# optuna/optuna

Hardware: NVIDIA H100
Metric: TPE suggestions/sec at 100k-trial history, 32 params (higher is better)
Workload: dtype f64

## Files before the change

### optuna_b200/csrc/tpe_kernels.cuh

```cuda
#pragma once
#include <cooperative_groups.h>

#include <type_traits>

#include "tpe_common.cuh"
#include "tpe_math.cuh"
#include "mt_jump_table.inc"

namespace tpe {

__global__ void k_rowok(const double* __restrict__ X, int64_t n, int32_t pall, const ColMeta* __restrict__ cols,
                        int32_t pc, uint8_t* __restrict__ ok) {
  for (int64_t i = blockIdx.x * (int64_t)blockDim.x + threadIdx.x; i < n; i += (int64_t)gridDim.x * blockDim.x) {
    bool good = true;
    for (int j = 0; j < pc; ++j) {
      const double v = X[i * pall + cols[j].src];
      good = good && (v == v);
    }
    ok[i] = good ? 1 : 0;
  }
}

struct SplitWork {
  int cat_count[4];
// ... 1102 lines not shown
  __device__ __forceinline__ void push_sync(double L) {
    const bool hit = L > thr;
    b3 = hit ? b2 : b3;
    b2 = hit ? b1 : b2;
    b1 = hit ? b0 : b1;
    b0 = hit ? L : b0;
    cnt += hit ? 1 : 0;
    if (__any_sync(0xffffffffu, cnt == 4)) flush();
  }
};

template <int PB, int PS, int RC, int NT, int TK, int ST, bool PAIR, int MINB>
__global__ void __launch_bounds__(NT, MINB)
k_logpdf_fast(const void* __restrict__ tab_v, const double* __restrict__ cst, int64_t Kf,
              const double2* __restrict__ colprm, const double* __restrict__ xT, int64_t ct_stride, int64_t kps,
              double lse_skip, double2* __restrict__ part) {
  static_assert(PB % PS == 0 && RC % PS == 0, "bad tiling");
  static_assert(!PAIR || PS == 1, "PAIR tables are not split over lanes");
  constexpr int PL = PB / PS;
  constexpr int RL = RC / PS;
  constexpr int GW = 32 / PS;
  constexpr int CW = GW * RC;
  using Elem = typename std::conditional<PAIR, double2, double>::type;
  constexpr int ES = PAIR ? 16 : 8;
  extern __shared__ __align__(128) unsigned char smem_raw[];
  Elem* tiles = reinterpret_cast<Elem*>(smem_raw);
  double* csts = reinterpret_cast<double*>(smem_raw + (size_t)ST * TK * PB * ES);
  uint64_t* full = reinterpret_cast<uint64_t*>(csts + (size_t)ST * TK);
  const Elem* tab = reinterpret_cast<const Elem*>(tab_v);
  const int tid = threadIdx.x;
  const int lane = tid & 31;
  const int h = lane % PS;
  const int g = lane / PS;
  const int64_t k0 = blockIdx.y * kps;
  const int64_t k1 = (k0 + kps < Kf) ? k0 + kps : Kf;
  const int ntiles = (k1 > k0) ? (int)((k1 - k0 + TK - 1) / TK) : 0;
  const int64_t wbase = (int64_t)blockIdx.x * ((NT / 32) * CW) + (int64_t)(tid >> 5) * CW;

  if (tid == 0) {
    for (int s = 0; s < ST; ++s) mbar_init(&full[s], 1);
    mbar_fence_init();
    LseAcc::skip() = lse_skip;
  }
  __syncthreads();

  auto issue = [&](int t) {
    const int st = t % ST;
    const int64_t ks = k0 + (int64_t)t * TK;
    const int tk = (int)((k1 - ks < TK) ? (k1 - ks) : TK);
    const uint32_t b_tile = (uint32_t)(((size_t)tk * PB * ES + 15) & ~(size_t)15);
    const uint32_t b_cst = (uint32_t)(((tk + 1) & ~1) * 8);
    fence_proxy_async();
    mbar_expect_tx(&full[st], b_tile + b_cst);
    bulk_g2s(tiles + (size_t)st * TK * PB, tab + ks * PB, b_tile, &full[st]);
    bulk_g2s(csts + (size_t)st * TK, cst + ks, b_cst, &full[st]);
  };
  if (tid == 0) {
    for (int t = 0; t < ST - 1 && t < ntiles; ++t) issue(t);
  }

  double x[RC][PL];
#pragma unroll
  for (int p = 0; p < PL; ++p) {
    const int slot = (PL == 1) ? h : 2 * ((p >> 1) * PS + h) + (p & 1);
    const double2 cp = colprm[slot];
#pragma unroll
    for (int r = 0; r < RC; ++r) {
      const int64_t ct = wbase + (int64_t)r * GW + g;
      x[r][p] = (xT[(int64_t)slot * ct_stride + ct] - cp.x) * cp.y;
    }
  }
  LseAcc acc[RL];
#pragma unroll
  for (int r = 0; r < RL; ++r) acc[r].init();

  for (int t = 0; t < ntiles; ++t) {
    const int st = t % ST;
    if (tid == 0 && t + ST - 1 < ntiles) issue(t + ST - 1);
    mbar_wait(&full[st], (uint32_t)((t / ST) & 1));
    const int64_t ks = k0 + (int64_t)t * TK;
    const int tk = (int)((k1 - ks < TK) ? (k1 - ks) : TK);
    const Elem* tile = tiles + (size_t)st * TK * PB;
    const double* ctile = csts + (size_t)st * TK;
    for (int kk = 0; kk < tk; ++kk) {
      double a0[RC], a1[RC];
#pragma unroll
      for (int r = 0; r < RC; ++r) {
        a0[r] = 0.0;
        a1[r] = 0.0;
      }
      if constexpr (PAIR) {
        const double2* row = reinterpret_cast<const double2*>(tile) + (size_t)kk * PB;
#pragma unroll
        for (int p = 0; p < PL; ++p) {
          const double2 v = row[p];
#pragma unroll
          for (int r = 0; r < RC; ++r) {
            const double d = fma(x[r][p], v.y, -v.x);
            if (p & 1) a1[r] = fma(d, d, a1[r]);
            else a0[r] = fma(d, d, a0[r]);
          }
        }
      } else if constexpr (PL == 1) {
        const double v = reinterpret_cast<const double*>(tile)[(size_t)kk * PB + h];
#pragma unroll
        for (int r = 0; r < RC; ++r) {
          const double d = x[r][0] - v;
          a0[r] = d * d;
        }
      } else {
        const double2* row =
            reinterpret_cast<const double2*>(reinterpret_cast<const double*>(tile) + (size_t)kk * PB) + h;
#pragma unroll
        for (int q = 0; q < PL / 2; ++q) {
          const double2 v = row[q * PS];
#pragma unroll
          for (int r = 0; r < RC; ++r) {
            const double d0 = x[r][2 * q] - v.x;
            const double d1 = x[r][2 * q + 1] - v.y;
            a0[r] = fma(d0, d0, a0[r]);
            a1[r] = fma(d1, d1, a1[r]);
          }
        }
      }
      double sum[RC];
#pragma unroll
      for (int r = 0; r < RC; ++r) sum[r] = a0[r] + a1[r];
      if constexpr (PS == 2) {
#pragma unroll
        for (int r = 0; r < RL; ++r) {
          const double mine = h ? sum[RL + r] : sum[r];
          const double send = h ? sum[r] : sum[RL + r];
          sum[r] = mine + __shfl_xor_sync(0xffffffffu, send, 1);
        }
      } else if constexpr (PS == 4) {
        double half[RC / 2];
#pragma unroll
        for (int r = 0; r < RC / 2; ++r) {
          const double mine = (h & 2) ? sum[RC / 2 + r] : sum[r];
          const double send = (h & 2) ? sum[r] : sum[RC / 2 + r];
          half[r] = mine + __shfl_xor_sync(0xffffffffu, send, 2);
        }
#pragma unroll
        for (int r = 0; r < RL; ++r) {
          const double mine = (h & 1) ? half[RL + r] : half[r];
          const double send = (h & 1) ? half[r] : half[RL + r];
          sum[r] = mine + __shfl_xor_sync(0xffffffffu, send, 1);
        }
      }
      const double c = ctile[kk];
#pragma unroll
      for (int r = 0; r < RL; ++r) acc[r].push_sync(fma(-0.5, sum[r], c));
    }
    __syncthreads();
  }
#pragma unroll
  for (int r = 0; r < RL; ++r) acc[r].flush();
#pragma unroll
  for (int r = 0; r < RL; ++r) {
    const int64_t ct = wbase + (int64_t)(h * RL + r) * GW + g;
    part[blockIdx.y * ct_stride + ct] = make_double2(acc[r].m, acc[r].s);
  }
}

__device__ __forceinline__ float ex2_approx(float x) {
  float y;
  asm("ex2.approx.ftz.f32 %0, %1;" : "=f"(y) : "f"(x));
  return y;
}
__device__ __forceinline__ double uni_exp(double x, const double* __restrict__ tab64) {
  const double t = fma(x, 92.332482616893656768, 6755399441055744.0);
  const int ni = __double2loint(t);
  const double nf = t - 6755399441055744.0;
  double r = fma(nf, -1.08304246932675596327e-02, x);
  r = fma(nf, -2.98158582698529328128e-12, r);
  double p = 8.33333333333333333333e-03;
  p = fma(p, r, 4.16666666666666666667e-02);
  p = fma(p, r, 1.66666666666666666667e-01);
  p = fma(p, r, 0.5);
  p = fma(p, r, 1.0);
  p = fma(p, r, 1.0);
  const double y = tab64[ni & 63] * p;
  return __hiloint2double(__double2hiint(y) + ((ni >> 6) << 20), __double2loint(y));
}

constexpr double kRefMove = 48.0;
__device__ __forceinline__ unsigned long long ld_relaxed_gpu(const unsigned long long* p) {
  unsigned long long v;
  asm volatile("ld.relaxed.gpu.global.u64 %0, [%1];" : "=l"(v) : "l"(p));
  return v;
}
struct LseRef {
  double R, s, base;
  float ffar;
  float thn;
  unsigned wp;
  __device__ __forceinline__ void init(unsigned slot0) {
    R = -INFINITY; s = 0.0; base = -INFINITY;
    ffar = 0.0f; thn = -INFINITY; wp = slot0;
  }
  __device__ __forceinline__ void rebase(double nb, float tnear, const double* e64) {
    if (__any_sync(0xffffffffu, nb > R + kRefMove)) {
      const bool mv = nb > R + kRefMove;
      const double f = uni_exp(fmax(R - nb, -700.0), e64);
      s = mv ? (s + (double)ffar) * f : s;
      ffar = mv ? 0.0f : ffar;
      R = mv ? nb : R;
    }
    base = nb;
    const float d = __double2float_rn(base - R);
    thn = (R == -INFINITY) ? -INFINITY : d - tnear;
  }
  template <int RS>
  __device__ __forceinline__ void flush(const double* ring, float tnear, const double* e64) {
    const unsigned slot0 = (unsigned)__cvta_generic_to_shared(ring);
    const int cnt = parked<RS>(slot0);
    const int n = __reduce_max_sync(0xffffffffu, cnt);
    double nb = base;
    for (int i = 0; i < n; ++i) {
      const double v = ring[i * RS];
      nb = (i < cnt && v > nb) ? v : nb;
    }
    rebase(nb, tnear, e64);
    double sum = 0.0;
    for (int i = 0; i < n; ++i) {
      const double e = uni_exp(fmax(ring[i * RS] - R, -700.0), e64);
      sum += (i < cnt) ? e : 0.0;
    }
    s += sum;
    wp = slot0;
  }
  template <int RS>
  __device__ __forceinline__ void park(double L, bool near) {
    asm volatile("{\n\t.reg .pred p;\n\tsetp.ne.u32 p, %2, 0;\n\t@p st.shared.f64 [%0], %1;\n\t}"
                 :: "r"(wp), "d"(L), "r"((unsigned)near) : "memory");
    wp += near ? RS * 8 : 0;
  }
  template <int RS>
  __device__ __forceinline__ int parked(unsigned slot0) const { return (int)((wp - slot0) / (RS * 8)); }
  __device__ __forceinline__ void roll() {
    s += (double)ffar;
    ffar = 0.0f;
  }
  __device__ __forceinline__ void sync_global(unsigned long long* slot, unsigned long long& pend, float tnear,
                                              const double* e64) {
    const double seen = from_order_bits(pend);
    pend = ld_relaxed_gpu(slot);
    if (base > seen) atomicMax(slot, static_cast<unsigned long long>(order_bits(base)));
    if (__any_sync(0xffffffffu, seen > base)) rebase(fmax(base, seen), tnear, e64);
  }
  __device__ __forceinline__ bool classify(double L, float gap, float& add, int& nfar) const {
    const float df = __double2float_rn(L - R);
    const bool near = df > thn;
    const bool far = !near && df > thn - gap;
    const float e = ex2_approx(df * 1.44269504f);
    add += far ? e : 0.0f;
    nfar += far ? 1 : 0;
    return near;
  }
  __device__ __forceinline__ double2 result(const double* e64) const {
    return make_double2(base, s * uni_exp(fmax(R - base, -700.0), e64));
  }
};

__device__ __forceinline__ void dmma_8x8x4(double& d0, double& d1, double a, double b) {
  asm volatile("mma.sync.aligned.m8n8k4.row.col.f64.f64.f64.f64 {%0,%1}, {%2}, {%3}, {%0,%1};"
               : "+d"(d0), "+d"(d1)
               : "d"(a), "d"(b));
}
__device__ __forceinline__ void dmma_16x8x8(double& d0, double& d1, double& d2, double& d3, double a0, double a1,
                                            double a2, double a3, double b0, double b1) {
  asm volatile("mma.sync.aligned.m16n8k8.row.col.f64.f64.f64.f64 {%0,%1,%2,%3}, {%4,%5,%6,%7}, {%8,%9}, {%0,%1,%2,%3};"
               : "+d"(d0), "+d"(d1), "+d"(d2), "+d"(d3)
               : "d"(a0), "d"(a1), "d"(a2), "d"(a3), "d"(b0), "d"(b1));
}
template <int PB, int M, int KG, int NT, int TK, int ST, int MINB>
struct MmaSmem {
  static constexpr size_t stages = (size_t)ST * TK * PB * 8 + (size_t)ST * TK * 8 + (size_t)ST * 16;
  static constexpr int NVG = 2 * KG;
  static constexpr int RS = (NT / 32) * M * 32;
  static constexpr size_t kSm = 228 * 1024, kCta = 1024 + 64 * 8;
  static constexpr size_t ctas_ = kSm / (stages + kCta);
  static constexpr size_t ctas = ctas_ < (size_t)MINB ? ctas_ : (size_t)MINB;
  static constexpr size_t fit = (kSm / ctas - kCta - stages) / (RS * 8);
  static constexpr int cap = (2 * NVG > 8) ? 2 * NVG : 8;
  static constexpr int D = (fit < (size_t)cap) ? (int)fit : cap;
  static_assert(D >= NVG, "the near-term ring does not fit beside the TMA stages: fewer stages or a shorter tile");
  static constexpr size_t bytes = stages + (size_t)D * RS * 8;
};

#ifdef TPE_LAB
__device__ unsigned long long g_mma_lab_count[5];
#endif

template <int PB, int M, int KG, int NT, int TK, int ST, int MINB, int DBG = 0>
__global__ void __launch_bounds__(NT, MINB)
k_logpdf_mma(const double* __restrict__ tabm, const double* __restrict__ ckk, int64_t Kfp,
             const double2* __restrict__ colprm, const double* __restrict__ xT, int64_t ct_stride, int64_t kps,
             double lse_skip, double2* __restrict__ part, unsigned long long* __restrict__ gmax,
             double lse_near) {
  static_assert(PB % 8 == 0 && TK % (8 * KG) == 0 && (M == 1 || M % 2 == 0), "bad tiling");
  constexpr int NI = PB / 4;
  constexpr int CW = 8 * M;
  extern __shared__ __align__(128) unsigned char smem_raw[];
  __shared__ double s_e64[64];
  double* tiles = reinterpret_cast<double*>(smem_raw);
  double* csts = tiles + (size_t)ST * TK * PB;
  uint64_t* full = reinterpret_cast<uint64_t*>(csts + (size_t)ST * TK);
  uint64_t* empty = full + ST;
  using SM = MmaSmem<PB, M, KG, NT, TK, ST, MINB>;
  double* ring = reinterpret_cast<double*>(empty + ST) + (threadIdx.x >> 5) * M * 32 + (threadIdx.x & 31);
  const int tid = threadIdx.x;
  const int lane = tid & 31;
  const int g = lane >> 2, q = lane & 3;
  const int64_t k0 = blockIdx.y * kps;
  const int64_t k1 = (k0 + kps < Kfp) ? k0 + kps : Kfp;
  const int ntiles = (k1 > k0) ? (int)((k1 - k0 + TK - 1) / TK) : 0;
  const int nsteps = (k1 > k0) ? (int)((k1 - k0) / (8 * KG)) : 0;
  const int64_t wbase = (int64_t)blockIdx.x * ((NT / 32) * CW) + (int64_t)(tid >> 5) * CW;

  if (tid < 64) s_e64[tid] = exp2((double)tid * 0.015625);
  if (tid == 0) {
    for (int s = 0; s < ST; ++s) {
      mbar_init(&full[s], 1);
      mbar_init(&empty[s], NT / 32);
    }
    mbar_fence_init();
  }
  __syncthreads();
  auto issue = [&](int t) {
    const int st = t % ST;
    const int64_t ks = k0 + (int64_t)t * TK;
    const int tk = (int)((k1 - ks < TK) ? (k1 - ks) : TK);
    const uint32_t b_tile = (uint32_t)((size_t)tk * PB * 8);
    const uint32_t b_cst = (uint32_t)(tk * 8);
    fence_proxy_async();
    mbar_expect_tx(&full[st], b_tile + b_cst);
    bulk_g2s(tiles + (size_t)st * TK * PB, tabm + ks * PB, b_tile, &full[st]);
    bulk_g2s(csts + (size_t)st * TK, ckk + ks, b_cst, &full[st]);
  };
  if (tid == 0) {
    for (int t = 0; t < ST - 1 && t < ntiles; ++t) issue(t);
  }
  auto enter = [&](int t) {
    if (tid == 0 && t + ST - 1 < ntiles) {
      if (t > 0) mbar_wait(&empty[(t - 1) % ST], (uint32_t)(((t - 1) / ST) & 1));
      issue(t + ST - 1);
    }
    mbar_wait(&full[t % ST], (uint32_t)((t / ST) & 1));
  };
  auto groups_in = [&](int t) {
    const int64_t ks = k0 + (int64_t)t * TK;
    return (int)((k1 - ks < TK) ? (k1 - ks) : TK) / 8;
  };

  double a[M][NI];
  double ha[M];
#pragma unroll
  for (int m = 0; m < M; ++m) ha[m] = 0.0;
#pragma unroll
  for (int i = 0; i < NI; ++i) {
    const int slot = 4 * i + q;
    const double2 cp = colprm[slot];
#pragma unroll
    for (int m = 0; m < M; ++m) {
      const int64_t ct = wbase + 8 * m + g;
      const double v = (xT[(int64_t)slot * ct_stride + ct] - cp.x) * cp.y;
      a[m][i] = v;
      ha[m] = fma(v, v, ha[m]);
    }
  }
#pragma unroll
  for (int m = 0; m < M; ++m) {
    ha[m] += __shfl_xor_sync(0xffffffffu, ha[m], 1);
    ha[m] += __shfl_xor_sync(0xffffffffu, ha[m], 2);
    ha[m] *= -0.5;
  }

  constexpr int NL = (M % 2 == 0) ? NI / 2 : NI;
  auto chain = [&](int t, int kg, double (&d)[KG][M][2], auto&& work) {
    const double* tile = tiles + (size_t)(t % ST) * TK * PB;
    const double* ctile = csts + (size_t)(t % ST) * TK;
    const double2* fb = reinterpret_cast<const double2*>(tile + (size_t)kg * 8 * PB) + lane;
#pragma unroll
    for (int u = 0; u < KG; ++u) {
      const double2 cc = reinterpret_cast<const double2*>(ctile + (kg + u) * 8)[q];
#pragma unroll
      for (int m = 0; m < M; ++m) {
        d[u][m][0] = cc.x;
        d[u][m][1] = cc.y;
      }
    }
    double2 v[2][KG];
#pragma unroll
    for (int u = 0; u < KG; ++u) v[0][u] = fb[u * (4 * PB)];
#pragma unroll
    for (int i2 = 0; i2 < NI / 2; ++i2) {
      if (i2 + 1 < NI / 2) {
#pragma unroll
        for (int u = 0; u < KG; ++u) v[(i2 + 1) & 1][u] = fb[u * (4 * PB) + (i2 + 1) * 32];
      }
      if constexpr (M % 2 == 0) {
#pragma unroll
        for (int u = 0; u < KG; ++u)
#pragma unroll
          for (int m = 0; m < M; m += 2)
            dmma_16x8x8(d[u][m][0], d[u][m][1], d[u][m + 1][0], d[u][m + 1][1], a[m][2 * i2], a[m + 1][2 * i2],
                        a[m][2 * i2 + 1], a[m + 1][2 * i2 + 1], v[i2 & 1][u].x, v[i2 & 1][u].y);
        work(i2);
      } else {
#pragma unroll
        for (int u = 0; u < KG; ++u) dmma_8x8x4(d[u][0][0], d[u][0][1], a[0][2 * i2], v[i2 & 1][u].x);
        work(2 * i2);
#pragma unroll
        for (int u = 0; u < KG; ++u) dmma_8x8x4(d[u][0][0], d[u][0][1], a[0][2 * i2 + 1], v[i2 & 1][u].y);
        work(2 * i2 + 1);
      }
    }
  };

  LseRef acc[M];
  unsigned long long gpend[M];
#pragma unroll
  for (int m = 0; m < M; ++m) {
    acc[m].init((unsigned)__cvta_generic_to_shared(ring + m * 32));
    gpend[m] = ld_relaxed_gpu(gmax + wbase + 8 * m + g);
  }
  const float lim_near = (float)lse_near, lim_gap = (float)(lse_skip - lse_near);
  int lab_far = 0;
  unsigned lab_near = 0, lab_flush = 0, lab_occ = 0, lab_walk = 0;

  constexpr int NV = 2 * KG * M;
  double cur[KG][M][2], nxt[KG][M][2];
  int tc = 0, kc = 0;
  int ngc = 0;
  auto none = [](int) {};
  if (nsteps > 0) {
    enter(0);
    ngc = groups_in(0);
    chain(0, 0, cur, none);
  }
  for (int s = 0; s < nsteps; ++s) {
    if constexpr (DBG != 4) {
      if (kc == 0 || tc == 0) {
#pragma unroll
        for (int m = 0; m < M; ++m) {
          acc[m].roll();
          acc[m].sync_global(gmax + wbase + 8 * m + g, gpend[m], lim_near, s_e64);
        }
      } else if ((kc & 15) == 0) {
#pragma unroll
        for (int m = 0; m < M; ++m) acc[m].roll();
      }
    }
    bool nr[M][2 * KG];
    float add[M];
#pragma unroll
    for (int m = 0; m < M; ++m) add[m] = 0.0f;
    auto cls = [&](int j) {
      const int m = j / (2 * KG), u = (j % (2 * KG)) / 2, h = j & 1;
      if constexpr (DBG == 1 || DBG == 4) acc[m].s += cur[u][m][h];
      else nr[m][j % (2 * KG)] = acc[m].classify(cur[u][m][h], lim_gap, add[m], lab_far);
    };
    auto work = [&](int i) {
#pragma unroll
      for (int j = 0; j < NV; ++j)
        if (j * NL / NV == i) cls(j);
    };

    int tn = tc, kn = kc + KG, ngn = ngc;
    if (kn == ngc) {
      __syncwarp();
      if (lane == 0) mbar_arrive(&empty[tc % ST]);
      tn = tc + 1;
      kn = 0;
      if (tn < ntiles) {
        enter(tn);
        ngn = groups_in(tn);
      }
    }
    if (s + 1 < nsteps) {
      chain(tn, kn, nxt, work);
    } else {
#pragma unroll
      for (int j = 0; j < NV; ++j) cls(j);
    }

    if constexpr (DBG != 1 && DBG != 4) {
#pragma unroll
      for (int m = 0; m < M; ++m) {
        acc[m].ffar += add[m];
        if constexpr (DBG == 0 || DBG == 5) {
#pragma unroll
          for (int i = 0; i < 2 * KG; ++i) {
            acc[m].template park<SM::RS>(cur[i / 2][m][i % 2], nr[m][i]);
            if constexpr (DBG == 5) lab_near += nr[m][i] ? 1 : 0;
          }
          const unsigned slot0 = (unsigned)__cvta_generic_to_shared(ring + m * 32);
          if (__any_sync(0xffffffffu, acc[m].wp > slot0 + (SM::D - SM::NVG) * SM::RS * 8)) {
            if constexpr (DBG == 5) {
              const int cnt = acc[m].template parked<SM::RS>(slot0);
              lab_flush += 1;
              lab_occ += cnt;
              lab_walk += __reduce_max_sync(0xffffffffu, cnt);
            }
            acc[m].template flush<SM::RS>(ring + m * 32, lim_near, s_e64);
          }
        }
      }
    }
#pragma unroll
    for (int u = 0; u < KG; ++u)
#pragma unroll
      for (int m = 0; m < M; ++m) {
        cur[u][m][0] = nxt[u][m][0];
        cur[u][m][1] = nxt[u][m][1];
      }
    tc = tn;
    kc = kn;
    ngc = ngn;
  }
#pragma unroll
  for (int m = 0; m < M; ++m) {
    acc[m].template flush<SM::RS>(ring + m * 32, lim_near, s_e64);
    acc[m].roll();
    const double2 r = acc[m].result(s_e64);
    double mm = r.x, ss = r.y;
#pragma unroll
    for (int o = 1; o <= 2; o <<= 1) {
      const double m2 = __shfl_xor_sync(0xffffffffu, mm, o), s2 = __shfl_xor_sync(0xffffffffu, ss, o);
      lse_merge(m2, s2, mm, ss);
    }
    if (q == 0) part[blockIdx.y * ct_stride + wbase + 8 * m + g] = make_double2(mm + ha[m], ss);
  }
#ifdef TPE_LAB
  if constexpr (DBG == 5) {
    const unsigned nn = __reduce_add_sync(0xffffffffu, lab_near);
    const unsigned nf = __reduce_add_sync(0xffffffffu, (unsigned)lab_far);
    const unsigned no = __reduce_add_sync(0xffffffffu, lab_occ);
    if (lane == 0) {
      atomicAdd(&g_mma_lab_count[0], (unsigned long long)nn);
      atomicAdd(&g_mma_lab_count[1], (unsigned long long)nf);
      atomicAdd(&g_mma_lab_count[2], (unsigned long long)lab_flush);
      atomicAdd(&g_mma_lab_count[3], (unsigned long long)no);
      atomicAdd(&g_mma_lab_count[4], (unsigned long long)lab_walk);
    }
  }
#endif
}

__device__ __forceinline__ void d_acq(const double2* __restrict__ part_l, int nsl, const double2* __restrict__ part_g, int nsg,
                      int64_t ct_stride, const uint8_t* __restrict__ oob, const double2* __restrict__ fix_l,
                      const double2* __restrict__ fix_g, int64_t Ct, double* __restrict__ logl,
                      double* __restrict__ logg) {
  const int lane = threadIdx.x & 31;
  const int64_t warp = (blockIdx.x * (int64_t)blockDim.x + threadIdx.x) >> 5;
  const int64_t nwarps = ((int64_t)gridDim.x * blockDim.x) >> 5;
  for (int64_t ct = warp; ct < Ct; ct += nwarps) {
    double ml = -INFINITY, sl = 0.0, mg = -INFINITY, sg = 0.0;
    if (oob != nullptr && oob[ct]) {
      ml = fix_l[ct].x; sl = fix_l[ct].y;
      mg = fix_g[ct].x; sg = fix_g[ct].y;
    } else {
      for (int s = lane; s < nsl; s += 32) {
        const double2 v = part_l[(int64_t)s * ct_stride + ct];
        lse_merge(v.x, v.y, ml, sl);
      }
      for (int s = lane; s < nsg; s += 32) {
        const double2 v = part_g[(int64_t)s * ct_stride + ct];
        lse_merge(v.x, v.y, mg, sg);
      }
#pragma unroll
      for (int o = 16; o > 0; o >>= 1) {
        const double m2 = __shfl_xor_sync(0xffffffffu, ml, o), s2 = __shfl_xor_sync(0xffffffffu, sl, o);
        lse_merge(m2, s2, ml, sl);
        const double m3 = __shfl_xor_sync(0xffffffffu, mg, o), s3 = __shfl_xor_sync(0xffffffffu, sg, o);
        lse_merge(m3, s3, mg, sg);
      }
    }
    if (lane == 0) {
      logl[ct] = (ml == -INFINITY) ? -INFINITY : log(sl) + ml;
      logg[ct] = (mg == -INFINITY) ? -INFINITY : log(sg) + mg;
    }
  }
}
__global__ void
k_acq(const double2* __restrict__ part_l, int nsl, const double2* __restrict__ part_g, int nsg,
                      int64_t ct_stride, const uint8_t* __restrict__ oob, const double2* __restrict__ fix_l,
                      const double2* __restrict__ fix_g, int64_t Ct, double* __restrict__ logl,
                      double* __restrict__ logg) { d_acq(part_l, nsl, part_g, nsg, ct_stride, oob, fix_l, fix_g, Ct, logl, logg); }

__global__ void k_reduce_parts(const double2* __restrict__ part, int ns, int64_t ct_stride, int64_t Ct,
                               double2* __restrict__ out) {
  for (int64_t ct = blockIdx.x * (int64_t)blockDim.x + threadIdx.x; ct < Ct; ct += (int64_t)gridDim.x * blockDim.x) {
    double m = -INFINITY, s = 0.0;
    for (int i = 0; i < ns; ++i) {
      const double2 v = part[(int64_t)i * ct_stride + ct];
      lse_merge(v.x, v.y, m, s);
    }
    out[ct] = make_double2(m, s);
  }
}

__device__ __forceinline__ void d_select(const double* __restrict__ logl, const double* __restrict__ logg, int32_t C, const double* __restrict__ S,
         int32_t pc, double* __restrict__ out_x, double* __restrict__ out_acq, int64_t* __restrict__ out_best) {
  __shared__ double s_val[256];
  __shared__ int s_idx[256];
  const int64_t ask = blockIdx.x;
  const int tid = threadIdx.x;
  double best = 0.0;
  int besti = -1;
  bool best_nan = false;
  for (int c = tid; c < C; c += 256) {
    const int64_t ct = ask * C + c;
    const double a = logl[ct] - logg[ct];
    const bool a_nan = a != a;
    if (besti < 0 || (!best_nan && (a_nan || a > best))) {
      best = a;
      besti = c;
      best_nan = a_nan;
    }
  }
  s_val[tid] = best;
  s_idx[tid] = besti;
  __syncthreads();
  for (int o = 128; o > 0; o >>= 1) {
    if (tid < o) {
      const double a = s_val[tid], b = s_val[tid + o];
      const int ia = s_idx[tid], ib = s_idx[tid + o];
      bool take_b;
      if (ib < 0) take_b = false;
      else if (ia < 0) take_b = true;
      else {
        const bool an = a != a, bn = b != b;
        if (an && bn) take_b = ib < ia;
        else if (an) take_b = false;
        else if (bn) take_b = true;
        else take_b = (b > a) || (b == a && ib < ia);
      }
      if (take_b) {
        s_val[tid] = b;
        s_idx[tid] = ib;
      }
    }
    __syncthreads();
  }
  const int bi = s_idx[0];
  if (tid == 0) {
    if (out_best) out_best[ask] = bi;
    if (out_acq) out_acq[ask] = s_val[0];
  }
  for (int j = tid; j < pc; j += 256) out_x[ask * pc + j] = S[(ask * C + bi) * pc + j];
}
__global__ void __launch_bounds__(256)
k_select(const double* __restrict__ logl, const double* __restrict__ logg, int32_t C, const double* __restrict__ S,
         int32_t pc, double* __restrict__ out_x, double* __restrict__ out_acq, int64_t* __restrict__ out_best) { d_select(logl, logg, C, S, pc, out_x, out_acq, out_best); }

__global__ void k_finish_logpdf(const double2* __restrict__ part, int ns, int64_t ct_stride,
                                const uint8_t* __restrict__ oob, const double2* __restrict__ fix, int64_t n,
                                double* __restrict__ out) {
  for (int64_t ct = blockIdx.x * (int64_t)blockDim.x + threadIdx.x; ct < n; ct += (int64_t)gridDim.x * blockDim.x) {
    double m = -INFINITY, s = 0.0;
    if (oob != nullptr && oob[ct]) {
      m = fix[ct].x;
      s = fix[ct].y;
    } else {
      for (int i = 0; i < ns; ++i) {
        const double2 v = part[(int64_t)i * ct_stride + ct];
        lse_merge(v.x, v.y, m, s);
      }
    }
    out[ct] = (m == -INFINITY) ? -INFINITY : log(s) + m;
  }
}

__device__ __forceinline__ uint32_t mt_temper(uint32_t y) {
  y ^= y >> 11;
  y ^= (y << 7) & 0x9d2c5680u;
  y ^= (y << 15) & 0xefc60000u;
  y ^= y >> 18;
  return y;
}
__device__ __forceinline__ uint32_t mt_twist(uint32_t cur, uint32_t nxt, uint32_t far) {
  const uint32_t y = (cur & 0x80000000u) | (nxt & 0x7fffffffu);
  return far ^ (y >> 1) ^ ((y & 1u) ? 0x9908b0dfu : 0u);
}
constexpr int kMtThreads = 768;
__device__ __forceinline__ void mt_gen_barrier() { asm volatile("bar.sync 1, 256;" ::: "memory"); }
__global__ void __launch_bounds__(kMtThreads, 1)
k_mt19937_uniform(uint32_t* __restrict__ key, int* __restrict__ pos_io, int64_t skip, int64_t count,
                  double* __restrict__ out) {
  __shared__ uint32_t buf[2][624];
  __shared__ uint32_t carry;
  const int tid = threadIdx.x;
  const bool gen = tid < 256;
  const int wt = tid - 256;
  for (int i = tid; i < 624; i += kMtThreads) buf[0][i] = key[i];
  int cur = 0;
  int start = *pos_io;
  int64_t gw = 0;
  const int64_t total_words = 2 * (skip + count);
  int end_pos = start;
  __syncthreads();
  {
    const int64_t drop_words = 2 * skip;
    int blocks = 0;
    if (gw + (624 - start) <= drop_words && gw + (624 - start) < total_words) {
      blocks = 1 + (int)((drop_words - (gw + (624 - start))) / 624);
      while (blocks > 0 && gw + (624 - start) + (int64_t)(blocks - 1) * 624 >= total_words) --blocks;
    }
    if (blocks > 0) {
      if (gen) {
        for (int bl = 0; bl < blocks; ++bl) {
          const uint32_t* A = buf[(cur + bl) & 1];
          uint32_t* B = buf[(cur + bl + 1) & 1];
          if (tid < 227) B[tid] = mt_twist(A[tid], A[tid + 1], A[tid + 397]);
          mt_gen_barrier();
          if (tid < 227) B[227 + tid] = mt_twist(A[227 + tid], A[228 + tid], B[tid]);
          mt_gen_barrier();
          if (tid < 170) {
            const int j = 454 + tid;
            B[j] = mt_twist(A[j], (j == 623) ? B[0] : A[j + 1], B[j - 227]);
          }
          mt_gen_barrier();
        }
      }
      gw += (624 - start) + (int64_t)(blocks - 1) * 624;
      cur = (cur + blocks) & 1;
      start = 0;
      end_pos = 0;
      __syncthreads();
    }
  }
  while (gw < total_words) {
    const int64_t avail = 624 - start;
    const int take = (int)((total_words - gw < avail) ? (total_words - gw) : avail);
    const bool more = gw + take < total_words;
    const uint32_t* A = buf[cur];
    uint32_t* B = buf[cur ^ 1];
    if (gen) {
      if (more) {
        if (tid < 227) B[tid] = mt_twist(A[tid], A[tid + 1], A[tid + 397]);
        mt_gen_barrier();
        if (tid < 227) B[227 + tid] = mt_twist(A[227 + tid], A[228 + tid], B[tid]);
        mt_gen_barrier();
        if (tid < 170) {
          const int j = 454 + tid;
          B[j] = mt_twist(A[j], (j == 623) ? B[0] : A[j + 1], B[j - 227]);
        }
      }
    } else {
      const int odd = (int)(gw & 1);
      if (odd && wt == 0 && take > 0) {
        const int64_t d = gw >> 1;
        const uint32_t a = carry, b2 = mt_temper(A[start]) >> 6;
        if (d >= skip) out[d - skip] = ((double)a * 67108864.0 + (double)b2) / 9007199254740992.0;
      }
      const int pairs = (take - odd) / 2;
      for (int p = wt; p < pairs; p += 512) {
        const int j = start + odd + 2 * p;
        const int64_t d = (gw + odd) / 2 + p;
        const uint32_t a = mt_temper(A[j]) >> 5, b2 = mt_temper(A[j + 1]) >> 6;
        if (d >= skip) out[d - skip] = ((double)a * 67108864.0 + (double)b2) / 9007199254740992.0;
      }
    }
    __syncthreads();
    if (tid == 256 && take > 0 && ((take - (int)(gw & 1)) & 1)) carry = mt_temper(A[start + take - 1]) >> 5;
    gw += take;
    if (more) {
      cur ^= 1;
      start = 0;
      end_pos = 0;
    } else {
      end_pos = start + take;
    }
  }
  __syncthreads();
  for (int i = tid; i < 624; i += kMtThreads) key[i] = buf[cur][i];
  if (tid == 0) *pos_io = end_pos;
}

constexpr int kMtJumpWords = 33 * 624;
constexpr int kMtJumpPad = 64;
constexpr int kMtJumpOut = 20;
constexpr size_t kMtJumpSmem = (size_t)(4 + kMtJumpWords + kMtJumpPad) * 4 + (size_t)24 * 640 * 4 + 2 * 624 * 4 + 16;

__device__ __forceinline__ void mt_next_block(const uint32_t* A, uint32_t* B, int tid) {
  if (tid < 227) B[tid] = mt_twist(A[tid], A[tid + 1], A[tid + 397]);
  mt_gen_barrier();
  if (tid < 227) B[227 + tid] = mt_twist(A[227 + tid], A[228 + tid], B[tid]);
  mt_gen_barrier();
  if (tid < 170) {
    const int j = 454 + tid;
    B[j] = mt_twist(A[j], (j == 623) ? B[0] : A[j + 1], B[j - 227]);
  }
  mt_gen_barrier();
}

__device__ __forceinline__ void mt_jump_apply(uint32_t* W, uint32_t* red, const uint32_t* __restrict__ g) {
  const int tid = threadIdx.x, lane = tid & 31, warp = tid >> 5;
  if (tid < 256)
    for (int b = 1; b < 33; ++b) mt_next_block(W + 624 * (b - 1), W + 624 * b, tid);
  __syncthreads();
  uint32_t acc[kMtJumpOut];
#pragma unroll
  for (int q = 0; q < kMtJumpOut; ++q) acc[q] = 0u;
  for (int ib = warp; ib < 624; ib += 24) {
    const uint32_t G = __ldg(g + ib);
    if (G == 0u) continue;
    uint32_t win[52];
    const uint4* src = reinterpret_cast<const uint4*>(W + 1 + 32 * ib + kMtJumpOut * lane);
#pragma unroll
    for (int v = 0; v < 13; ++v) {
      const uint4 x = src[v];
      win[4 * v] = x.x; win[4 * v + 1] = x.y; win[4 * v + 2] = x.z; win[4 * v + 3] = x.w;
    }
#pragma unroll
    for (int t = 0; t < 32; ++t) {
      if ((G >> t) & 1u) {
#pragma unroll
        for (int q = 0; q < kMtJumpOut; ++q) acc[q] ^= win[t + q];
      }
    }
// ... 119 lines not shown
```

Measured before the change: 709.8.

## Replace empty mbarriers with last-warp-issues atomic release and ping-pong step buffers

The TMA refill is no longer done by thread 0 waiting on an empty mbarrier. Each warp now atomically increments a per-stage shared counter, and whichever warp arrives last issues the refill, so no thread blocks on slower warps. All ST stages are prefetched up front. The step loop is unrolled by two with ping-pong register buffers, which removes the per-step cur=nxt copies and moves tile-crossing checks to every other step. This requires an even number of steps per tile, and a shortened final tile in the slice may break the pairing assumption.

```diff
diff --git a/optuna_b200/csrc/tpe_kernels.cuh b/optuna_b200/csrc/tpe_kernels.cuh
--- a/optuna_b200/csrc/tpe_kernels.cuh
+++ b/optuna_b200/csrc/tpe_kernels.cuh
@@ -1428,14 +1428,17 @@
   static_assert(PB % 8 == 0 && TK % (8 * KG) == 0 && (M == 1 || M % 2 == 0), "bad tiling");
   constexpr int NI = PB / 4;
   constexpr int CW = 8 * M;
+  constexpr int NW = NT / 32;
+  constexpr int NS = TK / (8 * KG);
+  static_assert(NS % 2 == 0, "the step loop runs two steps at a time and crosses tiles only between pairs");
   extern __shared__ __align__(128) unsigned char smem_raw[];
   __shared__ double s_e64[64];
   double* tiles = reinterpret_cast<double*>(smem_raw);
   double* csts = tiles + (size_t)ST * TK * PB;
   uint64_t* full = reinterpret_cast<uint64_t*>(csts + (size_t)ST * TK);
-  uint64_t* empty = full + ST;
+  unsigned long long* rel = reinterpret_cast<unsigned long long*>(full + ST);
   using SM = MmaSmem<PB, M, KG, NT, TK, ST, MINB>;
-  double* ring = reinterpret_cast<double*>(empty + ST) + (threadIdx.x >> 5) * M * 32 + (threadIdx.x & 31);
+  double* ring = reinterpret_cast<double*>(rel + ST) + (threadIdx.x >> 5) * M * 32 + (threadIdx.x & 31);
   const int tid = threadIdx.x;
   const int lane = tid & 31;
   const int g = lane >> 2, q = lane & 3;
@@ -1449,7 +1452,7 @@
   if (tid == 0) {
     for (int s = 0; s < ST; ++s) {
       mbar_init(&full[s], 1);
-      mbar_init(&empty[s], NT / 32);
+      rel[s] = 0;
     }
     mbar_fence_init();
   }
@@ -1466,15 +1469,18 @@
     bulk_g2s(csts + (size_t)st * TK, ckk + ks, b_cst, &full[st]);
   };
   if (tid == 0) {
-    for (int t = 0; t < ST - 1 && t < ntiles; ++t) issue(t);
-  }
-  auto enter = [&](int t) {
-    if (tid == 0 && t + ST - 1 < ntiles) {
-      if (t > 0) mbar_wait(&empty[(t - 1) % ST], (uint32_t)(((t - 1) / ST) & 1));
-      issue(t + ST - 1);
-    }
-    mbar_wait(&full[t % ST], (uint32_t)((t / ST) & 1));
+    for (int t = 0; t < ST && t < ntiles; ++t) issue(t);
+  }
+  auto release = [&](int t) {
+    __syncwarp();
+    if (lane == 0) {
+      unsigned long long n;
+      asm volatile("atom.acq_rel.cta.shared::cta.add.u64 %0, [%1], 1;"
+                   : "=l"(n) : "r"(smem_u32(&rel[t % ST])) : "memory");
+      if (n % NW == NW - 1) issue(t + ST);
+    }
   };
+  auto enter = [&](int t) { mbar_wait(&full[t % ST], (uint32_t)((t / ST) & 1)); };
   auto groups_in = [&](int t) {
     const int64_t ks = k0 + (int64_t)t * TK;
     return (int)((k1 - ks < TK) ? (k1 - ks) : TK) / 8;
@@ -1557,60 +1563,36 @@
   unsigned lab_near = 0, lab_flush = 0, lab_occ = 0, lab_walk = 0;
 
   constexpr int NV = 2 * KG * M;
-  double cur[KG][M][2], nxt[KG][M][2];
-  int tc = 0, kc = 0;
-  int ngc = 0;
-  auto none = [](int) {};
-  if (nsteps > 0) {
-    enter(0);
-    ngc = groups_in(0);
-    chain(0, 0, cur, none);
-  }
-  for (int s = 0; s < nsteps; ++s) {
+  auto pre = [&](int t, int kg) {
     if constexpr (DBG != 4) {
-      if (kc == 0 || tc == 0) {
+      if (kg == 0 || t == 0) {
 #pragma unroll
         for (int m = 0; m < M; ++m) {
           acc[m].roll();
           acc[m].sync_global(gmax + wbase + 8 * m + g, gpend[m], lim_near, s_e64);
         }
-      } else if ((kc & 15) == 0) {
+      } else if (NS * KG > 16 && (kg & 15) == 0) {
 #pragma unroll
         for (int m = 0; m < M; ++m) acc[m].roll();
       }
     }
+  };
+  auto step = [&](double (&c)[KG][M][2], int tn, int kn, double (&n)[KG][M][2]) {
     bool nr[M][2 * KG];
     float add[M];
 #pragma unroll
     for (int m = 0; m < M; ++m) add[m] = 0.0f;
     auto cls = [&](int j) {
       const int m = j / (2 * KG), u = (j % (2 * KG)) / 2, h = j & 1;
-      if constexpr (DBG == 1 || DBG == 4) acc[m].s += cur[u][m][h];
-      else nr[m][j % (2 * KG)] = acc[m].classify(cur[u][m][h], lim_gap, add[m], lab_far);
+      if constexpr (DBG == 1 || DBG == 4) acc[m].s += c[u][m][h];
+      else nr[m][j % (2 * KG)] = acc[m].classify(c[u][m][h], lim_gap, add[m], lab_far);
     };
     auto work = [&](int i) {
 #pragma unroll
       for (int j = 0; j < NV; ++j)
         if (j * NL / NV == i) cls(j);
     };
-
-    int tn = tc, kn = kc + KG, ngn = ngc;
-    if (kn == ngc) {
-      __syncwarp();
-      if (lane == 0) mbar_arrive(&empty[tc % ST]);
-      tn = tc + 1;
-      kn = 0;
-      if (tn < ntiles) {
-        enter(tn);
-        ngn = groups_in(tn);
-      }
-    }
-    if (s + 1 < nsteps) {
-      chain(tn, kn, nxt, work);
-    } else {
-#pragma unroll
-      for (int j = 0; j < NV; ++j) cls(j);
-    }
+    chain(tn, kn, n, work);
 
     if constexpr (DBG != 1 && DBG != 4) {
 #pragma unroll
@@ -1619,7 +1601,7 @@
         if constexpr (DBG == 0 || DBG == 5) {
 #pragma unroll
           for (int i = 0; i < 2 * KG; ++i) {
-            acc[m].template park<SM::RS>(cur[i / 2][m][i % 2], nr[m][i]);
+            acc[m].template park<SM::RS>(c[i / 2][m][i % 2], nr[m][i]);
             if constexpr (DBG == 5) lab_near += nr[m][i] ? 1 : 0;
           }
           const unsigned slot0 = (unsigned)__cvta_generic_to_shared(ring + m * 32);
@@ -1635,16 +1617,36 @@
         }
       }
     }
-#pragma unroll
-    for (int u = 0; u < KG; ++u)
-#pragma unroll
-      for (int m = 0; m < M; ++m) {
-        cur[u][m][0] = nxt[u][m][0];
-        cur[u][m][1] = nxt[u][m][1];
-      }
-    tc = tn;
-    kc = kn;
-    ngc = ngn;
+  };
+
+  double ca[KG][M][2], cb[KG][M][2];
+  int t = 0, kg = 0, ng = 0;
+  if (nsteps > 0) {
+    enter(0);
+    ng = groups_in(0);
+    chain(0, 0, ca, [](int) {});
+  }
+  for (int s = 0; s < nsteps; s += 2) {
+    const bool two = s + 1 < nsteps;
+    pre(t, kg);
+    step(ca, t, two ? kg + KG : kg, cb);
+    if (!two) break;
+    kg += KG;
+    pre(t, kg);
+    int tn = t, kn = kg + KG;
+    if (kn == ng) {
+      if (t + ST < ntiles) release(t);
+      tn = t + 1;
+      kn = 0;
+      if (tn < ntiles) {
+        enter(tn);
+        ng = groups_in(tn);
+      }
+    }
+    const bool more = s + 2 < nsteps;
+    step(cb, more ? tn : t, more ? kn : kg, ca);
+    t = tn;
+    kg = kn;
   }
 #pragma unroll
   for (int m = 0; m < M; ++m) {
```

Measured after the change: 778.3 (median of 6 runs). 9.7% higher.
